# zyang1580/SML

Measured on AMD Instinct MI355X. Metric: SML retrain-period training triples/s (MF + transfer stages), Yelp-shaped synthetic, d=32, higher is better.
Workload: dtype f32; 1 GPU; yelp_period: users=60000 items=123000 interactions/period=75000 neg=999 d=32 multi_num=10 MF_batch=1024 TR_batch=256 val_eval=True (the reference's 40 validation evaluations per period: 31 computed on the GPU, 9 memoised because the tables did not change in between -- identical numbers); MF stage: the transfer net runs once per DISTINCT row of a batch (the reference gathers one row per occurrence:; parallelism=single GPU

## Files before the change

sml_amd/csrc/transfer_fwd_body.inc:

```
    constexpr int R = SML_TM * MT;
    constexpr int K1 = SML_C2 * D;
    constexpr int HL = SML_HID / NS / HSEQ;
    constexpr int S1 = K1 + 4;
    constexpr int S2 = HL + 4;
    constexpr int KS1 = K1 / 16;
    constexpr int EPT = R * D / 512;
    constexpr int JT = D / 16;
    constexpr int CT = HL / 16 / 8;
    constexpr int KL = HL / 16;
    constexpr int KSPL = (D == 32) ? 8 : (D == 64 ? 4 : 2);
    constexpr int JSPL = 8 / KSPL;
    constexpr int JTW = JT / JSPL;
    constexpr int KPW = KL / KSPL;
    static_assert(CT >= 1 && KPW >= 1 && MT * NS <= 4 && (R * D) % 512 == 0, "tiling");
    constexpr int REG0 = cmax(R * S1, KSPL * R * (D + 1));
    __shared__ __attribute__((aligned(16))) float smem[REG0 + cmax(R * S2, R * (D + 1) + R) + 104];
    __shared__ SmlSched swin[SML_SW];
    __shared__ SmlReplayEnt rtab[MT == 1 ? SML_RP_N : 1];
    float* A1s = smem;
    float* a2s = smem + REG0;
    float* cws = smem + REG0 + cmax(R * S2, R * (D + 1) + R);
    float* xts = a2s;
    float* nrm = a2s + R * (D + 1);
    float* part = smem;

    const int tid = threadIdx.x, lane = tid & 63, wv = tid >> 6, l15 = lane & 15, g4 = lane >> 4;
    TL_BEGIN(NS == 4 ? 1 : 4); TL_PREV();
    constexpr int WT_LOCAL = (NS == 4) ? SML_WT_FWD : SML_WT_FWD_LOCAL;
    int tile, h;
    if constexpr (NS == 4) {
        const int x = (int)blockIdx.x % 8;
        h = x / 2; tile = 2 * ((int)blockIdx.x / 8) + (x % 2);
        if (tile >= a.tiles_total) return;
// ... 2 lines not shown
    const SmlSeg sg = sidx ? a.seg[1] : a.seg[0];
    const int row0 = (tile - (sidx ? a.tiles0 : 0)) * R;
    const float* __restrict__ theta = sg.theta;
    float cw_reg = 0.0f;
    constexpr bool CONVSTEP = (NS == 4 && MT == 1 && HSEQ == 1);
    const bool cstep = CONVSTEP && a.cs_in != nullptr;
    constexpr int CRG = 21, CC4 = SML_CG / 4;
    f32x4 cg_acc = {0.f, 0.f, 0.f, 0.f}, cgx[4];
    float cs_p = 0.f, cs_m = 0.f, cs_v = 0.f;
    const int cs_k = tid;
    const int cs_off = cs_k < 30 ? cs_k : cs_k < 40 ? cs_k + 2 : cs_k < 90 ? cs_k + 4 : cs_k + 6;
    const int cg_lo = sidx ? a.cg_split : 0, cg_hi = sidx ? a.cg_total : a.cg_split;
    int cg_t = 0;
    const bool cg_mine = CONVSTEP && cstep && a.cg_part != nullptr && tid < CRG * CC4;
    if (!cstep) { if (tid < 104) cw_reg = theta[tid]; }
    const bool lazy = sg.last_tab != nullptr;
    if (lazy) sched_window_load(swin, a.sched, a.cur_step - 1, tid);
    const bool closed = MT == 1 && lazy && a.sched_len > 0;
    if constexpr (MT == 1) { if (closed) replay_table_build(rtab, a.sched, a.sched_len, a.cur_step - 1, tid); }
    const bool saver = (h == 0);

    constexpr bool PRE = (CT == 1) && (KS1 / 2 <= 5) && HSEQ == 1;
    constexpr int PF2 = KPW < 4 ? KPW : 4;
    const f32x4* __restrict__ img1 = reinterpret_cast<const f32x4*>(sg.pk + sml_pk_p1(D));
    const f32x4* __restrict__ img2 = reinterpret_cast<const f32x4*>(sg.pk + sml_pk_p2(D));
    const int tile0 = h * (HL / 16) + wv * CT;
    const int kq = wv % KSPL, jq = wv / KSPL;
    auto t1 = [tile0](int) { return tile0; };
    auto k1 = [](int t) { return t * (KS1 / 2); };
    auto t2 = [jq](int t) { return jq * JTW + t; };
    auto nokofs = [](int) { return 0; };
// ... 27 lines not shown
        if (dense) {
            const int live = (int)sg.hdr[tile - (sidx ? a.tiles0 : 0)].nrows;
#pragma unroll
            for (int q = 0; q < EPT; ++q) {
                const int r = (q * 512 + tid) / D;
                const uint32_t trow = sg.drec[row0 + r].row;
                ok[q] = r < live;
                idx[q] = ok[q] ? (int64_t)trow : 0;
            }
            if (live == 0) return;
        } else {
#pragma unroll
            for (int q = 0; q < EPT; ++q) {
                const int row = row0 + (q * 512 + tid) / D;
                ok[q] = row < sg.n_rows;
                idx[q] = ok[q] ? seg_row_index(sg, row) : 0;
            }
        }
        if constexpr (CONVSTEP) {
            if (cstep) {
                if (tid < 95) {
                    const float* st_ = a.cs_in + (int64_t)sidx * 3 * SML_CG;
                    cs_p = st_[cs_k]; cs_m = st_[SML_CG + cs_k]; cs_v = st_[2 * SML_CG + cs_k];
                }
                if (cg_mine) {
                    const int rg = tid / CC4, c4 = tid % CC4;
                    cg_t = rg + (cg_lo > rg ? ((cg_lo - rg + CRG - 1) / CRG) * CRG : 0);
#pragma unroll
                    for (int u = 0; u < 4; ++u) {
                        const int t = cg_t + u * CRG;
                        cgx[u] = *reinterpret_cast<const f32x4*>(a.cg_part + (int64_t)(t < cg_hi ? t : cg_lo) * SML_CG + c4 * 4);
                    }
                }
                __builtin_amdgcn_sched_barrier(0);
            }
        }
#pragma unroll
        for (int q = 0; q < EPT; ++q) {
            const int w = (q * 512 + tid) % D;
            xt[q] = sg.xt_tab[idx[q] * D + w];
            xh[q] = sg.xh_tab[idx[q] * D + w];
        }
        float m[EPT], v[EPT];
        int from[EPT];
        if (lazy) {
#pragma unroll
            for (int q = 0; q < EPT; ++q) {
                const int w = (q * 512 + tid) % D;
                m[q] = sg.m_tab[idx[q] * D + w];
                v[q] = sg.v_tab[idx[q] * D + w];
                from[q] = sg.last_tab[idx[q]];
            }
        }
        if constexpr (PREW) {
            ring_preload<CT, 5>(ringw1, img1, KS1, 0, lane, tw, nokofs);
            ring_preload<JTW, PF2>(ringw2, img2, 32, h * KL + kq * KPW, lane, t2, nokofs);
        }
        if constexpr (CONVSTEP) {
            if (cstep) {
                __builtin_amdgcn_sched_barrier(0);
                float* P = smem;
                if (tid < CRG * CC4) {
                    const int rg = tid / CC4, c4 = tid % CC4;
                    if (cg_mine) {
#pragma unroll
                        for (int u = 0; u < 4; ++u) if (cg_t + u * CRG < cg_hi) cg_acc += cgx[u];
                        for (int t0 = cg_t + 4 * CRG; t0 < cg_hi; t0 += 4 * CRG) {
                            f32x4 x[4];
#pragma unroll
                            for (int u = 0; u < 4; ++u) {
                                const int t = t0 + u * CRG;
                                x[u] = *reinterpret_cast<const f32x4*>(a.cg_part + (int64_t)(t < cg_hi ? t : cg_lo) * SML_CG + c4 * 4);
                            }
#pragma unroll
                            for (int u = 0; u < 4; ++u) if (t0 + u * CRG < cg_hi) cg_acc += x[u];
                        }
                    }
                    *reinterpret_cast<f32x4*>(P + rg * SML_CG + c4 * 4) = cg_acc;
                }
                asm volatile("s_waitcnt lgkmcnt(0)\n\ts_barrier" ::: "memory");
                if (tid < 95) {
// ... 187 lines not shown
```

sml_amd/csrc/transfer_net.hip:

```cpp
#include <cstdlib>
#include "sml_dev.h"
#include "sml_kernels.h"

#ifdef SML_TIMELINE
__device__ long long* g_timeline = nullptr;
#ifndef SML_TL_SECOND
#define SML_TL_SECOND (gridDim.x - 1)
#endif
#define TL_BEGIN(KID) long long* tl_rec = nullptr; const int tl_all = 70000 + (KID) * 1024; { if (g_timeline && threadIdx.x == 0) g_timeline[tl_all + 512 + blockIdx.x] = wall_clock64(); } { long long* tl = g_timeline; if (tl && threadIdx.x == 0 && (blockIdx.x == 0 || blockIdx.x == SML_TL_SECOND)) { \
    const unsigned long long slot = atomicAdd(reinterpret_cast<unsigned long long*>(tl), 1ull); tl_rec = tl + 16 + slot * 16; tl_rec[0] = (KID) * 2 + (blockIdx.x != 0); tl_rec[1] = wall_clock64(); for (int q = 2; q < 16; ++q) tl_rec[q] = 0; } }
#define TL(i) do { if (tl_rec) tl_rec[(i)] = wall_clock64(); } while (0)
#define TL_DONE() do { long long* tl = g_timeline; if (tl && threadIdx.x == 0) { const long long now_ = wall_clock64(); \
    atomicMax(reinterpret_cast<unsigned long long*>(tl + 2), (unsigned long long)now_); tl[tl_all + blockIdx.x] = now_; } } while (0)
#define TL_PREV() do { if (tl_rec) tl_rec[8] = (long long)__hip_atomic_load(reinterpret_cast<unsigned long long*>(g_timeline + 2), __ATOMIC_RELAXED, __HIP_MEMORY_SCOPE_AGENT); } while (0)
#else
#define TL_BEGIN(KID) const int tl_all = 0; (void)tl_all; long long* const tl_rec = nullptr; (void)tl_rec
#define TL(i) do { } while (0)
#define TL_DONE() do { } while (0)
#define TL_PREV() do { } while (0)
#endif
#ifndef SML_WT_FWD
#define SML_WT_FWD 2
#endif
#ifndef SML_WT_BWD
// ... 34 lines not shown
    }
#pragma unroll
    for (int q = 0; q < SML_C2; ++q) {
        float s = cw[SML_OFF_C2B + q];
#pragma unroll
        for (int c = 0; c < SML_C1; ++c) s += cw[SML_OFF_C2W + q * SML_C1 + c] * o.h1[c];
        o.h2p[q] = s;
    }
}

__device__ __forceinline__ int64_t seg_row_index(const SmlSeg& s, int r) {
    if (s.tri == nullptr) return r;
    if (!s.is_item) return s.tri[(int64_t)r * 3];
    return r < s.B ? s.tri[(int64_t)r * 3 + 1] : s.tri[(int64_t)(r - s.B) * 3 + 2];
}

template <int NT, int PFD, typename TileOf, typename KOfs>
__device__ __forceinline__ void ring_preload(f32x4 (&ring)[PFD][NT], const f32x4* __restrict__ bimg, int ksteps_total, int ks0,
                                             int lane, TileOf tile_of, KOfs kofs) {
#pragma unroll
    for (int i = 0; i < PFD; ++i)
#pragma unroll
        for (int t = 0; t < NT; ++t) ring[i][t] = bimg[(tile_of(t) * ksteps_total + ks0 + kofs(t) + i) * 64 + lane];
    __builtin_amdgcn_sched_barrier(0x86);
}

template <int MT, int NT, int NK, int PFD, bool SPLITK, typename TileOf, typename KOfs>
__device__ __forceinline__ void mma16_ring(f32x4 (&acc)[MT][NT], f32x4 (&ring)[PFD][NT], const float* arow, int a_mt,
                                           const f32x4* __restrict__ bimg, int ksteps_total, int ks0, int lane,
                                           TileOf tile_of, KOfs kofs) {
// ... 67 lines not shown
constexpr int cmax(int a, int b) { return a > b ? a : b; }

#define SML_FWD_HOT_PARAMS const float* __restrict__ p_pk, const float* __restrict__ p_theta, const int64_t* __restrict__ p_tri,             \
                           const float* __restrict__ p_cs_in, const float* __restrict__ p_cg_part, int p_B, int p_n0, int p_tiles, int p_cg
#define SML_FWD_HOT_PATCH(a, D)                                                                                                               \
    (a).tiles0 = p_tiles & 0x7fffffff; (a).tiles_total = (p_tiles & 0x7fffffff) + (p_tiles < 0 ? (2 * p_B + SML_TM - 1) / SML_TM : 0);       \
    (a).cs_in = p_cs_in; (a).cg_part = p_cg_part; (a).cg_split = p_cg & 0x7fff; (a).cg_total = (p_cg >> 15) & 0xffff;                         \
    (a).seg[0].pk = p_pk; (a).seg[1].pk = p_pk + sml_pk_size(D); (a).seg[0].theta = p_theta; (a).seg[1].theta = p_theta + sml_net_size(D); \
    (a).seg[0].tri = p_tri; (a).seg[1].tri = p_tri; (a).seg[0].B = p_B; (a).seg[1].B = p_B; (a).seg[0].n_rows = p_n0;                        \
    (a).seg[1].n_rows = p_n0 == p_B ? 2 * p_B : ((2 * p_B + SML_TM - 1) / SML_TM) * SML_TM;                                                   \
    (a).seg[0].is_item = 0; (a).seg[1].is_item = 1
template <int D, int MT, int NS, int HSEQ = 1>
__global__ __launch_bounds__(512) __attribute__((amdgpu_waves_per_eu(HSEQ > 1 ? 4 : 2, HSEQ > 1 ? 4 : 2))) void k_transfer_fwd(SML_FWD_HOT_PARAMS, SmlFwdArgs a_in) {
    SmlFwdArgs a = a_in;
    SML_FWD_HOT_PATCH(a, D);
#include "transfer_fwd_body.inc"
}
template <int D>
__global__ __launch_bounds__(512) __attribute__((amdgpu_waves_per_eu(4, 4))) void k_side_transfer_fwd(SmlFwdArgs a) {
    constexpr int MT = 2, NS = 1, HSEQ = 2;
#include "transfer_fwd_body.inc"
}

typedef __bf16 bf16x8 __attribute__((ext_vector_type(8)));
__device__ __forceinline__ f32x4 mfma_bf(const uint4& a, const uint4& b, f32x4 c) {
    return __builtin_amdgcn_mfma_f32_16x16x32_bf16(__builtin_bit_cast(bf16x8, a), __builtin_bit_cast(bf16x8, b), c, 0, 0, 0);
}
__device__ __forceinline__ uint32_t bf16_rne(float x) {
    uint32_t u = __float_as_uint(x);
    u += 0x7fffu + ((u >> 16) & 1u);
    return u >> 16;
}
__device__ __forceinline__ void split3(float x, unsigned short& h, unsigned short& m, unsigned short& l) {
    const uint32_t a = bf16_rne(x);
    const float r1 = x - __uint_as_float(a << 16);
// ... 213 lines not shown
    __shared__ __attribute__((aligned(16))) unsigned short A2b[3][R][S2B];
    __shared__ float cws[104];
    __shared__ SmlSched swin[SML_SW];
    __shared__ SmlReplayEnt rtab[SML_RP_N];
    float* part = reinterpret_cast<float*>(&A2b[0][0][0]);
    static_assert(sizeof(A2b) >= 8 * R * (D + 1) * sizeof(float), "part fits");
    const int tid = threadIdx.x, lane = tid & 63, wv = tid >> 6, l15 = lane & 15, g4 = lane >> 4;
    const int tile = (int)blockIdx.x;
    const int sidx = tile >= a.tiles0;
    const SmlSeg sg = sidx ? a.seg[1] : a.seg[0];
    const int tl = tile - (sidx ? a.tiles0 : 0);
    const int row0 = tl * R;
    const float* __restrict__ theta = sg.theta;
    const unsigned short* __restrict__ p1x = pkx + (int64_t)sidx * sml_bx3_size(D) + sml_bx3_p1(D);
    const unsigned short* __restrict__ p2x = pkx + (int64_t)sidx * sml_bx3_size(D) + sml_bx3_p2(D);
    if (tid < 104) cws[tid] = theta[tid];
    const bool lazy = sg.last_tab != nullptr;
    if (lazy) sched_window_load(swin, a.sched, a.cur_step - 1, tid);
    const int r = tid / D, w = tid % D;
    bool ok; int64_t idx;
    if (sg.drec != nullptr) {
        const int live = (int)sg.hdr[tl].nrows;
        const uint32_t trow = sg.drec[row0 + r].row;
        ok = r < live; idx = ok ? (int64_t)trow : 0;
        if (live == 0) return;
    } else {
        ok = row0 + r < sg.n_rows;
        idx = ok ? seg_row_index(sg, row0 + r) : 0;
    }
    float xt = sg.xt_tab[idx * D + w], xh = sg.xh_tab[idx * D + w];
    float m = 0.0f, v = 0.0f; int from = -1;
    if (lazy) { m = sg.m_tab[idx * D + w]; v = sg.v_tab[idx * D + w]; from = sg.last_tab[idx]; }
    const bool closed = lazy && a.sched_len > 0;
    if (closed) replay_table_build(rtab, a.sched, a.sched_len, a.cur_step - 1, tid);
    uint4 bw[2][CT][3];
    auto load_b1 = [&](int ks, uint4 (&dst)[CT][3]) {
#pragma unroll
        for (int t = 0; t < CT; ++t)
#pragma unroll
            for (int p = 0; p < 3; ++p)
                dst[t][p] = *reinterpret_cast<const uint4*>(p1x + ((((int64_t)(wv * CT + t) * KS1 + ks) * 3 + p) * 64 + lane) * 8);
    };
    load_b1(0, bw[0]);
    float bias1[CT];
#pragma unroll
    for (int t = 0; t < CT; ++t) bias1[t] = theta[sml_off_f1b(D) + (wv * CT + t) * 16 + l15];
    const float bias2 = theta[sml_off_f2b(D) + w];
    __builtin_amdgcn_sched_barrier(0);
    if (!ok) { xt = 1.0f; xh = 0.0f; }
    float nr2 = xt * xt;
#pragma unroll
    for (int off = D / 2; off >= 1; off >>= 1) nr2 += __shfl_xor(nr2, off, 64);
    __syncthreads();
    if (lazy) {
        if (ok) adam_replay_t(xh, m, v, from, a.cur_step - 1, a.sched, swin, a.cur_step - 1, closed ? rtab : nullptr);
        if (sg.mrep != nullptr) {
            sg.mrep[(int64_t)(row0 + r) * D + w] = ok ? m : 0.0f;
            sg.vrep[(int64_t)(row0 + r) * D + w] = ok ? v : 0.0f;
        }
    }
    {
        const float xc = a.k2 ? 0.0f : (xt * xh) / sqrtf(nr2);
        Pro p;
        conv_prologue(cws, xt, xh, xc, p);
#pragma unroll
        for (int c = 0; c < SML_C2; ++c) {
            unsigned short h, mm, l;
// ... 210 lines not shown
    __shared__ __attribute__((aligned(16))) float Cs[DENSEOK ? SML_TILE_ENT * D : 4];
    __shared__ uint32_t rlen[16], rstart[17];
    __shared__ float Ps[DENSEOK ? 512 : 4];
    float* dZs = smem;
    float* dOs = smem + R * S2;
    float* part = smem;
    float* cws = smem + SZ;

    const int tid = threadIdx.x, lane = tid & 63, wv = tid >> 6, l15 = lane & 15, g4 = lane >> 4;
    TL_BEGIN(5); TL_PREV();
    const int sidx = (int)blockIdx.x >= p_tiles0;
    const SmlBwdSeg& sg = a.seg[sidx];
    const float* __restrict__ sg_theta = p_theta + (sidx ? sml_net_size(D) : 0);
    const int row0 = ((int)blockIdx.x - (sidx ? p_tiles0 : 0)) * R;
    if (p_world > 0 && (int)blockIdx.x >= p_tiles_live) { peer_signal(a.push); return; }
    if (tid < 104) cws[tid] = sg_theta[tid];
#ifndef SML_PREB
#define SML_PREB 0
#endif
    constexpr bool PREB = (SML_PREB != 0) && (MT == 1) && (D <= 32);
    const f32x4* __restrict__ p2b = reinterpret_cast<const f32x4*>(sg.pk + sml_pk_p2b(D));
    const f32x4* __restrict__ p1b = reinterpret_cast<const f32x4*>(sg.pk + sml_pk_p1b(D));
    auto tileA2 = [wv](int t) { return wv * 4 + t; };
    auto tileA1 = [wv](int t) { return (wv / KSPL) * 5 + t; };
    auto nokofs = [](int) { return 0; };
    f32x4 ringb2[PREB ? KSD : 1][4], ringb1[PREB ? 4 : 1][5];
    float zpre[PREB ? MT : 1][4][4];
    auto preload_operands = [&]() {
        if constexpr (PREB) {
            ring_preload<4, KSD>(ringb2, p2b, KSD, 0, lane, tileA2, nokofs);
            ring_preload<5, 4>(ringb1, p1b, 32, (wv % KSPL) * KPER, lane, tileA1, nokofs);
// ... 219 lines not shown
    }
    constexpr bool PRELOAD = (EPT == 1);
    float x0p = 0.f, x1p = 0.f, x2p = 0.f;
    if (PRELOAD) {
        const float* x = sg.xin + (int64_t)(row0 + tid / D) * 3 * D;
        x0p = x[tid % D]; x1p = x[D + tid % D]; x2p = x[2 * D + tid % D];
    }
    constexpr bool FUSABLE = D <= 64;
    const bool fused = FUSABLE && a.fu.slot_info != nullptr;
    FusedPre fpre;
    fpre.info = SML_SLOT_ONCE; fpre.trow = 0; fpre.m = fpre.v = 0.0f; fpre.r0 = make_uint4(0u, 0u, 0u, 0u); fpre.r1 = fpre.r0;
    if constexpr (FUSABLE && PRELOAD) {
        if (fused) fused_prefetch<D>(a, sidx, row0 + tid / D, tid % D, row0 + tid / D < sg.n_rows, fpre);
        if (dense) dense_prefetch<D>(a, sidx, row0 + tid / D, tid % D, tid / D < live, fpre);
    }
    __syncthreads();
    TL(2);
    {
        f32x4 acc[MT][4];
        zero_acc(acc);
        float z[MT][4][4];
#pragma unroll
        for (int t = 0; t < 4; ++t)
#pragma unroll
            for (int mt = 0; mt < MT; ++mt)
#pragma unroll
                for (int q = 0; q < 4; ++q)
                    z[mt][t][q] = PREB ? zpre[mt][t][q] : sg.z1[(int64_t)(row0 + mt * SML_TM + 4 * g4 + q) * SML_HID + (wv * 4 + t) * 16 + l15];
        if constexpr (PREB) mma16_ring<MT, 4, KSD, KSD, false>(acc, ringb2, dOs + l15 * SD + 4 * g4, SML_TM * SD, p2b, KSD, 0, lane, tileA2, nokofs);
        else mma16_rows<MT, 4, KSD, KSD>(acc, dOs + l15 * SD + 4 * g4, SML_TM * SD, p2b, KSD, 0, lane, tileA2);
// ... 346 lines not shown
        if (lane == 0) lred[wv] = v;
    }
    __syncthreads();
    if (tid == 0) {
        float sacc = 0.0f;
#pragma unroll
        for (int w8 = 0; w8 < 8; ++w8) sacc += lred[w8];
        a.loss_part[blockIdx.x] = sacc;
        TL(7);
    }
    TL_DONE();
}

template <int D>
__global__ __launch_bounds__(512) void k_tr_bwd_head(const float* __restrict__ p_out_all, const float* __restrict__ p_z1, const float* __restrict__ p_pk,
                                                     long long p_out_pstride, int p_B, int p_ioff, int p_tiles0, int p_tiles_total, int p_out_np, SmlBwdArgs a) {
    constexpr int R = SML_TM;
    constexpr int HS = 4;
    constexpr int SD = D + 4;
    constexpr int KSD = D / 16;
    constexpr int EPT = R * D / 512;
    static_assert(SML_HID / 16 / HS == 8, "one dA2 column tile per wave");
    __shared__ __attribute__((aligned(16))) float smem[cmax(R * SD, 3 * R * (D + 1))];
    __shared__ float cf[4][SML_TM];
    __shared__ float lred[8];
    float* dOs = smem;
    float* O3 = smem;
    const int tid = threadIdx.x, lane = tid & 63, wv = tid >> 6, l15 = lane & 15, g4 = lane >> 4;
    TL_BEGIN(2); TL_PREV();
    const int x8 = (int)blockIdx.x % 8;
    const int hs = x8 / 2, tile = 2 * ((int)blockIdx.x / 8) + (x8 % 2);
    if (tile >= p_tiles_total) return;
    const int sidx = tile >= p_tiles0;
    const SmlBwdSeg sg = sidx ? a.seg[1] : a.seg[0];
    const int row0 = (tile - (sidx ? p_tiles0 : 0)) * R;
    const int n_rows = sidx ? 2 * p_B : p_B;
    const float* __restrict__ z1_seg = p_z1 + (sidx ? (int64_t)p_ioff * SML_HID : 0);
    const f32x4* __restrict__ p2b = reinterpret_cast<const f32x4*>(p_pk + (sidx ? sml_pk_size(D) : 0) + sml_pk_p2b(D));
    const int ct = hs * 8 + wv;
    float vu[EPT][SML_FWD_NS], vi[EPT][SML_FWD_NS], vn[EPT][SML_FWD_NS];
#pragma unroll
    for (int q = 0; q < EPT; ++q) {
        const int e = q * 512 + tid, r = e / D, w = e % D;
        const int row = row0 + r;
        const bool inr = row < n_rows;
        const int t = !inr ? 0 : ((sidx && row >= p_B) ? row - p_B : row);
        const float* pu = p_out_all + (int64_t)t * D + w;
        const float* pi = p_out_all + (int64_t)(p_ioff + t) * D + w;
        const float* pn = p_out_all + (int64_t)(p_ioff + p_B + t) * D + w;
#pragma unroll
        for (int p = 0; p < SML_FWD_NS; ++p) {
            const int64_t po = (int64_t)min(p, p_out_np - 1) * p_out_pstride;
            vu[q][p] = pu[po]; vi[q][p] = pi[po]; vn[q][p] = pn[po];
        }
    }
    float z[4];
#pragma unroll
    for (int q = 0; q < 4; ++q) z[q] = z1_seg[(int64_t)(row0 + 4 * g4 + q) * SML_HID + ct * 16 + l15];
    f32x4 ring[KSD];
#pragma unroll
    for (int ks = 0; ks < KSD; ++ks) ring[ks] = p2b[(ct * KSD + ks) * 64 + lane];
    float ou[EPT], oi[EPT], on[EPT];
#pragma unroll
    for (int q = 0; q < EPT; ++q) {
        const int e = q * 512 + tid, r = e / D, w = e % D;
        const float inr = (row0 + r < n_rows) ? 1.0f : 0.0f;
        ou[q] = oi[q] = on[q] = 0.0f;
#pragma unroll
        for (int p = 0; p < SML_FWD_NS; ++p) {
            const float live = p < p_out_np ? inr : 0.0f;
            ou[q] += live * vu[q][p]; oi[q] += live * vi[q][p]; on[q] += live * vn[q][p];
        }
        if constexpr (D > 64) {
            O3[(0 * R + r) * (D + 1) + w] = ou[q];
            O3[(1 * R + r) * (D + 1) + w] = oi[q];
            O3[(2 * R + r) * (D + 1) + w] = on[q];
// ... 27 lines not shown
#pragma unroll
        for (int q = 0; q < EPT; ++q) {
            const int e = q * 512 + tid, r = e / D, w = e % D;
            const int row = row0 + r;
            float sp = ou[q] * oi[q], sn = ou[q] * on[q], uu = ou[q] * ou[q];
#pragma unroll
            for (int off = D / 2; off >= 1; off >>= 1) {
                sp += __shfl_xor(sp, off, 64); sn += __shfl_xor(sn, off, 64); uu += __shfl_xor(uu, off, 64);
            }
            float lt, d0, d1, inv_nu, cc;
            coeffs(sp, sn, uu, lt, d0, d1, inv_nu, cc);
            d0 *= a.scale; d1 *= a.scale;
            if (!sidx && hs == 0 && w == 0 && row < n_rows) lsum += lt * a.scale;
            const float g = dout_of(row, d0, d1, inv_nu, cc, ou[q], oi[q], on[q]);
            dOs[r * SD + w] = g;
            if (hs == 0) st_out<SML_WT_BWD>(&sg.dout[(int64_t)row * D + w], g);
        }
    } else {
        __syncthreads();
        if (tid < R) {
            float sp = 0.f, sn = 0.f, uu = 0.f;
#pragma unroll 8
            for (int w = 0; w < D; ++w) {
                const float u = O3[(0 * R + tid) * (D + 1) + w];
                sp += u * O3[(1 * R + tid) * (D + 1) + w];
                sn += u * O3[(2 * R + tid) * (D + 1) + w];
                uu += u * u;
            }
            float lt, d0, d1, inv_nu, cc;
            coeffs(sp, sn, uu, lt, d0, d1, inv_nu, cc);
            cf[0][tid] = d0 * a.scale; cf[1][tid] = d1 * a.scale; cf[2][tid] = inv_nu; cf[3][tid] = cc;
            if (!sidx && hs == 0 && row0 + tid < n_rows) lsum = lt * a.scale;
        }
        __syncthreads();
#pragma unroll
        for (int q = 0; q < EPT; ++q) {
            const int e = q * 512 + tid, r = e / D, w = e % D;
            const int row = row0 + r;
            const float g = dout_of(row, cf[0][r], cf[1][r], cf[2][r], cf[3][r], ou[q], oi[q], on[q]);
            dOs[r * SD + w] = g;
            if (hs == 0) st_out<SML_WT_BWD>(&sg.dout[(int64_t)row * D + w], g);
        }
    }
    __syncthreads();
    TL(2);
    {
        f32x4 acc = {0.f, 0.f, 0.f, 0.f};
#pragma unroll
        for (int ks = 0; ks < KSD; ++ks) {
            const f32x4 av = *reinterpret_cast<const f32x4*>(dOs + l15 * SD + 4 * g4 + ks * 16);
#pragma unroll
            for (int e = 0; e < 4; ++e) acc = mfma16(av[e], ring[ks][e], acc);
        }
        const int n = ct * 16 + l15;
#pragma unroll
        for (int q = 0; q < 4; ++q)
            st_out<SML_WT_BWD>(&sg.dz1[(int64_t)(row0 + 4 * g4 + q) * SML_HID + n], acc[q] * sml_gelu_grad(z[q]));
    }
    TL(3);
    {
        float v = lsum;
#pragma unroll
        for (int off = 32; off >= 1; off >>= 1) v += __shfl_xor(v, off, 64);
        if (lane == 0) lred[wv] = v;
    }
    __syncthreads();
    if (tid == 0) {
        float sacc = 0.0f;
#pragma unroll
        for (int w8 = 0; w8 < 8; ++w8) sacc += lred[w8];
        a.loss_part[tile * HS + hs] = sacc;
        TL(7);
    }
    TL_DONE();
}

template <int D>
__device__ __forceinline__ void pack_store(float* __restrict__ pk, int off, float p) {
    constexpr int K1 = SML_C2 * D;
    if (off >= SML_OFF_F1W && off < sml_off_f1b(D)) {
        const int n = (off - SML_OFF_F1W) / K1, k = (off - SML_OFF_F1W) % K1;
        pk[sml_pk_p1(D) + pk_pos(K1 / 16, n, k)] = p;
        pk[sml_pk_p1b(D) + pk_pos(SML_HID / 16, k, n)] = p;
    } else if (off >= sml_off_f2w(D) && off < sml_off_f2b(D)) {
        const int j = (off - sml_off_f2w(D)) / SML_HID, n = (off - sml_off_f2w(D)) % SML_HID;
        pk[sml_pk_p2(D) + pk_pos(SML_HID / 16, j, n)] = p;
        pk[sml_pk_p2b(D) + pk_pos(D / 16, n, j)] = p;
    }
}

#define SML_WG_TILE_SMEM (8 * 32 * 33 + 8 * 32 + 32 * 33)
template <int D>
__device__ __forceinline__ void wgrad_tile(const SmlWgArgs& a, const SmlWgSeg& sg, int xcd, int kk, float* smem_wg, long long* tl_rec) {
    constexpr int K1 = SML_C2 * D;
    constexpr int KT = K1 / 32;
    constexpr int JT = D / 32;
    constexpr int T1 = 16 * KT, T2 = JT * 16, TN = T1 + T2;
    constexpr int NS = sml_net_size(D);
    float* part = smem_wg;
    float* csum = smem_wg + 8 * 32 * 33;
    float* wt = csum + 8 * 32;
    const int tid = threadIdx.x, lane = tid & 63, wv = tid >> 6, l31 = lane & 31, hi = lane >> 5;
    const bool fuse = a.theta != nullptr;
    SmlSched sc; sc.step_size = a.step_size; sc.bc2_sqrt = a.bc2_sqrt;
    static_assert(TN % 8 == 0 && T2 == 16 * JT, "tile map");
    constexpr int PER = 2 * (KT + JT);
    const int net = 1 - kk / PER, rr = kk % PER;
    const bool is_w1 = rr < 2 * KT;
    int ti, tj;
    if (is_w1) { ti = 2 * xcd + rr / KT; tj = rr % KT; } else { tj = 2 * xcd + (rr - 2 * KT) / JT; ti = (rr - 2 * KT) % JT; }
    const float* __restrict__ Asrc = is_w1 ? sg.dz1 : sg.dout;
    const int lda = is_w1 ? SML_HID : D;
    const float* __restrict__ Bsrc = is_w1 ? sg.a1 : sg.a2;
    const int ldb = is_w1 ? K1 : SML_HID;
    const bool gelu_b = !is_w1 && a.gelu_b != 0;
    int woff[2];
    float wp[2] = {0.f, 0.f}, wm[2] = {0.f, 0.f}, wvv[2] = {0.f, 0.f};
#pragma unroll
    for (int q = 0; q < 2; ++q) {
        const int e = q * 512 + tid, i = e >> 5, j = e & 31;
        woff[q] = is_w1 ? SML_OFF_F1W + (ti * 32 + i) * K1 + tj * 32 + j
                        : sml_off_f2w(D) + (ti * 32 + i) * SML_HID + tj * 32 + j;
    }
    const bool has_bias = (tj == 0 && tid < 32);
    const int boff = is_w1 ? sml_off_f1b(D) + ti * 32 + tid : sml_off_f2b(D) + ti * 32 + tid;
    float bp = 0.f, bm = 0.f, bv2 = 0.f;
    f32x16 acc;
#pragma unroll
    for (int q = 0; q < 16; ++q) acc[q] = 0.0f;
    float colsum = 0.0f;
// ... 106 lines not shown
template <int D>
__global__ __launch_bounds__(512) __attribute__((amdgpu_waves_per_eu(4, 4))) void k_tr_wgrad2(const float* __restrict__ p_dz1, const float* __restrict__ p_a1,
        const float* __restrict__ p_dout, const float* __restrict__ p_a2, const float* __restrict__ p_pk_net, const float* __restrict__ p_xin, int p_B, int p_n_tail,
        SmlWgArgs a) {
    SmlWgSeg seg0 = a.seg[0], seg1 = a.seg[1];
    {
        const int64_t slot1 = (int64_t)SML_R * ((p_B + SML_R - 1) / SML_R);
        seg0.dz1 = p_dz1; seg1.dz1 = p_dz1 + slot1 * SML_HID;
        seg0.a1 = p_a1; seg1.a1 = p_a1 + slot1 * SML_C2 * D;
        seg0.dout = p_dout; seg1.dout = p_dout + slot1 * D;
        seg0.a2 = p_a2; seg1.a2 = p_a2 + slot1 * SML_HID;
        seg0.pk_net = p_pk_net; seg1.pk_net = p_pk_net + sml_pk_size(D);
        seg0.xin = p_xin; seg1.xin = p_xin + slot1 * 3 * D;
        seg0.n_rows = p_B; seg1.n_rows = 2 * p_B;
    }
    const int h_n_tail = p_n_tail, h_tiles0 = (p_B + SML_TM - 1) / SML_TM, h_tiles_total = h_tiles0 + (2 * p_B + SML_TM - 1) / SML_TM;
    constexpr int R = SML_TM;
    constexpr int CS = D / 16;
    constexpr int S2 = SML_HID + 4;
    constexpr int PSTR = SML_C2 * 16 + 1;
    constexpr int CGS = 20;
    constexpr int SZ0 = cmax(cmax(R * S2, 8 * R * PSTR), 2 * 256 * CGS);
    constexpr int TAIL_SMEM = SZ0 + 104 + 8 * 256;
    constexpr int NS = sml_net_size(D);
    __shared__ __attribute__((aligned(16))) float smem[cmax(TAIL_SMEM, SML_WG_TILE_SMEM)];
    __shared__ int s_last;
    TL_BEGIN(3); TL_PREV();
    const int tid = threadIdx.x, lane = tid & 63, wv = tid >> 6, l15 = lane & 15, g4 = lane >> 4;
    if ((int)blockIdx.x >= h_n_tail) {
        const int vb = (int)blockIdx.x - h_n_tail;
        const SmlWgSeg sgt = ((vb / 8) / (2 * (SML_C2 * D / 32 + D / 32))) ? SmlWgSeg(seg0) : SmlWgSeg(seg1);
        float* const smem_tile = smem + (vb * 3 - vb - vb - vb);
        wgrad_tile<D>(a, sgt, (int)blockIdx.x % 8, vb / 8, smem_tile, tl_rec);
        TL_DONE();
        return;
    }
    float* part = smem;
    float* cgA = smem;
    float* cgB = smem + 256 * CGS;
    float* cws = smem + SZ0;
    float* red = smem + SZ0 + 104;
    const int tb = (int)blockIdx.x;
    const int tile = tb / CS, cs = tb % CS;
    const bool live = tile < h_tiles_total;
    if (live) {
        const int sidx = tile >= h_tiles0;
        const SmlWgSeg sg = sidx ? seg1 : seg0;
        const int row0 = (tile - (sidx ? h_tiles0 : 0)) * R;
// ... 278 lines not shown
        else k_side_transfer_fwd<64><<<dim3(tiles_total), dim3(512), 0, st>>>(a);
        return hipGetLastError();
    }
    const SmlSeg& s0 = a.seg[0]; const SmlSeg& s1 = a.seg[1];
    const bool two = tiles_total > a.tiles0 && s1.n_rows > 0;
    const int tt = a.tiles_total > a.tiles0 ? a.tiles_total : a.tiles0;
    const int n1 = s0.n_rows == s0.B ? 2 * s0.B : ((2 * s0.B + SML_TM - 1) / SML_TM) * SML_TM;
    if ((s0.tri != nullptr && s0.is_item != 0) || a.cg_split < 0 || a.cg_split > 0x7fff || a.cg_total < 0 || a.cg_total > 0xffff ||
        a.tiles0 < 0 || (tt != a.tiles0 && tt != a.tiles0 + (2 * s0.B + SML_TM - 1) / SML_TM) ||
        (two && (s1.pk != s0.pk + sml_pk_size(d) || s1.theta != s0.theta + sml_net_size(d) || s1.tri != s0.tri || s1.B != s0.B || s1.n_rows != n1 ||
                 (s1.tri != nullptr && s1.is_item != 1))))
        return hipErrorInvalidValue;
#define SML_FWD_HOT_ARGS s0.pk, s0.theta, s0.tri, a.cs_in, a.cg_part, s0.B, s0.n_rows, (int)((unsigned)a.tiles0 | (tt != a.tiles0 ? 0x80000000u : 0u)), \
                         (a.cg_split | (a.cg_total << 15)), a
    if (mt == 1 && ns == 1) { SML_DISPATCH_D(d, k_transfer_fwd<DD, 1, 1><<<dim3(tiles_total), dim3(512), 0, st>>>(SML_FWD_HOT_ARGS)); }
    else if (mt == 1 && ns == 4) { SML_DISPATCH_D(d, k_transfer_fwd<DD, 1, 4><<<dim3(((tiles_total + 1) / 2) * 8), dim3(512), 0, st>>>(SML_FWD_HOT_ARGS)); }
    else if (mt == 1 && ns == 2) { SML_DISPATCH_D(d, k_transfer_fwd<DD, 1, 2><<<dim3(tiles_total * 2), dim3(512), 0, st>>>(SML_FWD_HOT_ARGS)); }
    else if (mt == 2 && ns == 1) {
        if (d == 32) k_transfer_fwd<32, 2, 1, 2><<<dim3(tiles_total), dim3(512), 0, st>>>(SML_FWD_HOT_ARGS);
        else if (d == 64) k_transfer_fwd<64, 2, 1, 2><<<dim3(tiles_total), dim3(512), 0, st>>>(SML_FWD_HOT_ARGS);
        else if (d == 128) k_transfer_fwd<128, 2, 1><<<dim3(tiles_total), dim3(512), 0, st>>>(SML_FWD_HOT_ARGS);
        else return hipErrorInvalidValue;
    }
    else return hipErrorInvalidValue;
#undef SML_FWD_HOT_ARGS
    return hipGetLastError();
}
hipError_t sml_launch_bwd(int d, int split, const SmlBwdArgs& a, int tiles_total, hipStream_t st) {
    if (tiles_total <= 0) return hipSuccess;
    if (split) {
// ... 1 lines not shown
        if (d == 32) k_transfer_bwd<32, true><<<dim3(grid), dim3(512), 0, st>>>(a);
        else if (d == 64) k_transfer_bwd<64, false><<<dim3(grid), dim3(512), 0, st>>>(a);
        else if (d == 128) k_transfer_bwd<128, false><<<dim3(grid), dim3(512), 0, st>>>(a);
        else return hipErrorInvalidValue;
    } else {
        if (a.seg[1].theta != a.seg[0].theta + sml_net_size(d)) return hipErrorInvalidValue;
        SML_DISPATCH_D(d, k_transfer_bwd_full<DD, 1><<<dim3(tiles_total), dim3(512), 0, st>>>(a.dn.hdr, a.dn.ent, a.seg[0].theta, a.out_all, a.tiles0, a.push.world,
                                                                                                a.tiles_live, a.B, a));
    }
    return hipGetLastError();
}
hipError_t sml_launch_tr_bwd_head(int d, const SmlBwdArgs& a, int tiles_total, hipStream_t st) {
    if (tiles_total <= 0) return hipSuccess;
    const SmlBwdSeg& s0 = a.seg[0]; const SmlBwdSeg& s1 = a.seg[1];
    if (s1.z1 != s0.z1 + (int64_t)a.ioff * SML_HID || s1.pk != s0.pk + sml_pk_size(d) || s0.n_rows != a.B || s1.n_rows != 2 * a.B ||
        s0.is_item != 0 || s1.is_item != 1)
        return hipErrorInvalidValue;
    SML_DISPATCH_D(d, k_tr_bwd_head<DD><<<dim3(((tiles_total + 1) / 2) * 8), dim3(512), 0, st>>>(a.out_all, a.seg[0].z1, a.seg[0].pk, (long long)a.out_pstride,
                                                                                                   a.B, a.ioff, a.tiles0, a.tiles_total, a.out_np, a));
    return hipGetLastError();
}
int sml_wgrad_tiles(int d) { return 2 * (16 * (SML_C2 * d / 32) + (d / 32) * 16); }
hipError_t sml_launch_tr_wgrad2(int d, const SmlWgArgs& a, hipStream_t st) {
    const int tiles = sml_wgrad_tiles(d);
    const SmlWgSeg& s0 = a.seg[0]; const SmlWgSeg& s1 = a.seg[1];
    const int B = s0.n_rows;
    const int64_t slot1 = (int64_t)SML_R * ((B + SML_R - 1) / SML_R);
    if (s1.n_rows != 2 * B || s1.dz1 != s0.dz1 + slot1 * SML_HID || s1.a1 != s0.a1 + slot1 * SML_C2 * d || s1.dout != s0.dout + slot1 * d ||
        s1.a2 != s0.a2 + slot1 * SML_HID || s1.pk_net != s0.pk_net + sml_pk_size(d) || s1.xin != s0.xin + slot1 * 3 * d ||
        a.tiles0 != (B + SML_TM - 1) / SML_TM || a.tiles_total != a.tiles0 + (2 * B + SML_TM - 1) / SML_TM)
        return hipErrorInvalidValue;
    SML_DISPATCH_D(d, k_tr_wgrad2<DD><<<dim3(a.n_tail + tiles), dim3(512), 0, st>>>(s0.dz1, s0.a1, s0.dout, s0.a2, s0.pk_net, s0.xin, B, a.n_tail, a));
    return hipGetLastError();
}
hipError_t sml_launch_theta_adam(int d, const SmlThetaAdamArgs& a, hipStream_t st) {
    const int n = 2 * sml_net_size(d) / 4;
    if (a.peer.world > 0) { SML_DISPATCH_D(d, k_theta_adam<DD, true><<<dim3((n + 255) / 256), dim3(256), 0, st>>>(a)); }
    else { SML_DISPATCH_D(d, k_theta_adam<DD, false><<<dim3((n + 255) / 256), dim3(256), 0, st>>>(a)); }
    return hipGetLastError();
}
__global__ __launch_bounds__(256) void k_conv_state_init(const float* __restrict__ theta, const float* __restrict__ m, const float* __restrict__ v,
                                                         int net_size, float* __restrict__ cs) {
    const int net = threadIdx.x >> 7, k = threadIdx.x & 127;
    if (k >= 95) return;
    const int off = k < 30 ? k : k < 40 ? k + 2 : k < 90 ? k + 4 : k + 6;
    const long long i = (long long)net * net_size + off;
    float* o = cs + net * 3 * SML_CG;
// ... 48 lines not shown
```

Before: 15.98 million triples/s.

## Add non-lazy transfer forward kernel and hoist scalar arg loads earlier

Adds a k_tr_fwd specialization used when neither segment has lazy Adam tables. It drops the replay table and schedule window, issues row-index and conv-state/cg-part loads unconditionally with dummy addresses so they are in flight early, and picks the result afterwards. It also packs kind, scale and gelu_b into scalar kernel parameters, and moves theta and schedule loads into registers so the shared-memory stores sit just before the barrier. The aim is to cut load latency and kernel-argument memory reads, at the cost of more code paths and some wasted speculative loads.

```diff
diff --git a/sml_amd/csrc/transfer_fwd_body.inc b/sml_amd/csrc/transfer_fwd_body.inc
--- a/sml_amd/csrc/transfer_fwd_body.inc
+++ b/sml_amd/csrc/transfer_fwd_body.inc
@@ -16,7 +16,7 @@
     constexpr int REG0 = cmax(R * S1, KSPL * R * (D + 1));
     __shared__ __attribute__((aligned(16))) float smem[REG0 + cmax(R * S2, R * (D + 1) + R) + 104];
     __shared__ SmlSched swin[SML_SW];
-    __shared__ SmlReplayEnt rtab[MT == 1 ? SML_RP_N : 1];
+    __shared__ SmlReplayEnt rtab[(MT == 1 && !NOLAZY) ? SML_RP_N : 1];
     float* A1s = smem;
     float* a2s = smem + REG0;
     float* cws = smem + REG0 + cmax(R * S2, R * (D + 1) + R);
@@ -49,7 +49,7 @@
     int cg_t = 0;
     const bool cg_mine = CONVSTEP && cstep && a.cg_part != nullptr && tid < CRG * CC4;
     if (!cstep) { if (tid < 104) cw_reg = theta[tid]; }
-    const bool lazy = sg.last_tab != nullptr;
+    const bool lazy = !NOLAZY && sg.last_tab != nullptr;
     if (lazy) sched_window_load(swin, a.sched, a.cur_step - 1, tid);
     const bool closed = MT == 1 && lazy && a.sched_len > 0;
     if constexpr (MT == 1) { if (closed) replay_table_build(rtab, a.sched, a.sched_len, a.cur_step - 1, tid); }
@@ -107,26 +107,32 @@
             for (int q = 0; q < EPT; ++q) {
                 const int row = row0 + (q * 512 + tid) / D;
                 ok[q] = row < sg.n_rows;
-                idx[q] = ok[q] ? seg_row_index(sg, row) : 0;
+                if constexpr (NOLAZY) idx[q] = seg_row_index_load(sg, ok[q] ? row : 0, reinterpret_cast<const int64_t*>(img1));
+                else idx[q] = ok[q] ? seg_row_index(sg, row) : 0;
             }
         }
         if constexpr (CONVSTEP) {
-            if (cstep) {
-                if (tid < 95) {
-                    const float* st_ = a.cs_in + (int64_t)sidx * 3 * SML_CG;
-                    cs_p = st_[cs_k]; cs_m = st_[SML_CG + cs_k]; cs_v = st_[2 * SML_CG + cs_k];
-                }
-                if (cg_mine) {
-                    const int rg = tid / CC4, c4 = tid % CC4;
-                    cg_t = rg + (cg_lo > rg ? ((cg_lo - rg + CRG - 1) / CRG) * CRG : 0);
-#pragma unroll
-                    for (int u = 0; u < 4; ++u) {
-                        const int t = cg_t + u * CRG;
-                        cgx[u] = *reinterpret_cast<const f32x4*>(a.cg_part + (int64_t)(t < cg_hi ? t : cg_lo) * SML_CG + c4 * 4);
-                    }
+            {
+                const bool cg_on = cstep && a.cg_part != nullptr && cg_hi > cg_lo;
+                const float* nowhere = reinterpret_cast<const float*>(img1);
+                const float* st_ = cstep ? a.cs_in + (int64_t)sidx * 3 * SML_CG : nowhere;
+                const int ck = min(cs_k, 94);
+                cs_p = st_[ck]; cs_m = st_[SML_CG + ck]; cs_v = st_[2 * SML_CG + ck];
+                const int rg = min(tid / CC4, CRG - 1), c4 = tid % CC4;
+                cg_t = rg + (cg_lo > rg ? ((cg_lo - rg + CRG - 1) / CRG) * CRG : 0);
+                const float* cgp = cg_on ? a.cg_part : nowhere;
+                const int hi_c = cg_on ? cg_hi : 0, lo_c = cg_on ? cg_lo : 0;
+#pragma unroll
+                for (int u = 0; u < 4; ++u) {
+                    const int t = cg_t + u * CRG;
+                    cgx[u] = *reinterpret_cast<const f32x4*>(cgp + (int64_t)(t < hi_c ? t : lo_c) * SML_CG + c4 * 4);
                 }
                 __builtin_amdgcn_sched_barrier(0);
             }
+        }
+        if constexpr (NOLAZY) {
+#pragma unroll
+            for (int q = 0; q < EPT; ++q) idx[q] = seg_row_index_pick(sg, ok[q] ? row0 + (q * 512 + tid) / D : 0, idx[q]);
         }
 #pragma unroll
         for (int q = 0; q < EPT; ++q) {
@@ -150,14 +156,15 @@
             ring_preload<JTW, PF2>(ringw2, img2, 32, h * KL + kq * KPW, lane, t2, nokofs);
         }
         if constexpr (CONVSTEP) {
+            __builtin_amdgcn_sched_barrier(0);
+#pragma unroll
+            for (int u = 0; u < 4; ++u) cg_acc = (cg_mine && cg_t + u * CRG < cg_hi) ? cg_acc + cgx[u] : cg_acc;
+            asm volatile("" : "+v"(cg_acc));
             if (cstep) {
-                __builtin_amdgcn_sched_barrier(0);
                 float* P = smem;
                 if (tid < CRG * CC4) {
                     const int rg = tid / CC4, c4 = tid % CC4;
                     if (cg_mine) {
-#pragma unroll
-                        for (int u = 0; u < 4; ++u) if (cg_t + u * CRG < cg_hi) cg_acc += cgx[u];
                         for (int t0 = cg_t + 4 * CRG; t0 < cg_hi; t0 += 4 * CRG) {
                             f32x4 x[4];
 #pragma unroll
diff --git a/sml_amd/csrc/transfer_net.hip b/sml_amd/csrc/transfer_net.hip
--- a/sml_amd/csrc/transfer_net.hip
+++ b/sml_amd/csrc/transfer_net.hip
@@ -72,6 +72,12 @@
     if (!s.is_item) return s.tri[(int64_t)r * 3];
     return r < s.B ? s.tri[(int64_t)r * 3 + 1] : s.tri[(int64_t)(r - s.B) * 3 + 2];
 }
+__device__ __forceinline__ int64_t seg_row_index_load(const SmlSeg& s, int r, const int64_t* somewhere) {
+    const bool id = s.tri == nullptr;
+    const int64_t o = !s.is_item ? (int64_t)r * 3 : (r < s.B ? (int64_t)r * 3 + 1 : (int64_t)(r - s.B) * 3 + 2);
+    return (id ? somewhere : s.tri)[id ? 0 : o];
+}
+__device__ __forceinline__ int64_t seg_row_index_pick(const SmlSeg& s, int r, int64_t loaded) { return s.tri == nullptr ? (int64_t)r : loaded; }
 
 template <int NT, int PFD, typename TileOf, typename KOfs>
 __device__ __forceinline__ void ring_preload(f32x4 (&ring)[PFD][NT], const f32x4* __restrict__ bimg, int ksteps_total, int ks0,
@@ -169,11 +175,21 @@
 __global__ __launch_bounds__(512) __attribute__((amdgpu_waves_per_eu(HSEQ > 1 ? 4 : 2, HSEQ > 1 ? 4 : 2))) void k_transfer_fwd(SML_FWD_HOT_PARAMS, SmlFwdArgs a_in) {
     SmlFwdArgs a = a_in;
     SML_FWD_HOT_PATCH(a, D);
+    constexpr bool NOLAZY = false;
+#include "transfer_fwd_body.inc"
+}
+template <int D>
+__global__ __launch_bounds__(512) __attribute__((amdgpu_waves_per_eu(2, 2))) void k_tr_fwd(SML_FWD_HOT_PARAMS, SmlFwdArgs a_in) {
+    SmlFwdArgs a = a_in;
+    SML_FWD_HOT_PATCH(a, D);
+    constexpr int MT = 1, NS = 4, HSEQ = 1;
+    constexpr bool NOLAZY = true;
 #include "transfer_fwd_body.inc"
 }
 template <int D>
 __global__ __launch_bounds__(512) __attribute__((amdgpu_waves_per_eu(4, 4))) void k_side_transfer_fwd(SmlFwdArgs a) {
     constexpr int MT = 2, NS = 1, HSEQ = 2;
+    constexpr bool NOLAZY = false;
 #include "transfer_fwd_body.inc"
 }
 
@@ -417,14 +433,17 @@
     const float* __restrict__ theta = sg.theta;
     const unsigned short* __restrict__ p1x = pkx + (int64_t)sidx * sml_bx3_size(D) + sml_bx3_p1(D);
     const unsigned short* __restrict__ p2x = pkx + (int64_t)sidx * sml_bx3_size(D) + sml_bx3_p2(D);
-    if (tid < 104) cws[tid] = theta[tid];
+    const float cw_reg = theta[tid < 104 ? tid : 103];
     const bool lazy = sg.last_tab != nullptr;
-    if (lazy) sched_window_load(swin, a.sched, a.cur_step - 1, tid);
+    const int sw_k = a.cur_step - SML_SW + (tid < SML_SW ? tid : SML_SW - 1);
+    SmlSched sw_reg; sw_reg.step_size = 0.0f; sw_reg.bc2_sqrt = 0.0f;
     const int r = tid / D, w = tid % D;
     bool ok; int64_t idx;
-    if (sg.drec != nullptr) {
-        const int live = (int)sg.hdr[tl].nrows;
-        const uint32_t trow = sg.drec[row0 + r].row;
+    const bool dn = sg.drec != nullptr;
+    int live = 0; uint32_t trow = 0;
+    if (dn) { live = (int)sg.hdr[tl].nrows; trow = sg.drec[row0 + r].row; }
+    if (lazy) sw_reg = a.sched[sw_k >= 0 ? sw_k : 0];
+    if (dn) {
         ok = r < live; idx = ok ? (int64_t)trow : 0;
         if (live == 0) return;
     } else {
@@ -454,6 +473,8 @@
     float nr2 = xt * xt;
 #pragma unroll
     for (int off = D / 2; off >= 1; off >>= 1) nr2 += __shfl_xor(nr2, off, 64);
+    if (tid < 104) cws[tid] = cw_reg;
+    if (lazy && tid < SML_SW && sw_k >= 0) swin[tid] = sw_reg;
     __syncthreads();
     if (lazy) {
         if (ok) adam_replay_t(xh, m, v, from, a.cur_step - 1, a.sched, swin, a.cur_step - 1, closed ? rtab : nullptr);
@@ -694,7 +715,7 @@
     const float* __restrict__ sg_theta = p_theta + (sidx ? sml_net_size(D) : 0);
     const int row0 = ((int)blockIdx.x - (sidx ? p_tiles0 : 0)) * R;
     if (p_world > 0 && (int)blockIdx.x >= p_tiles_live) { peer_signal(a.push); return; }
-    if (tid < 104) cws[tid] = sg_theta[tid];
+    const float cw_reg = sg_theta[tid < 104 ? tid : 103];
 #ifndef SML_PREB
 #define SML_PREB 0
 #endif
@@ -944,6 +965,7 @@
         if (fused) fused_prefetch<D>(a, sidx, row0 + tid / D, tid % D, row0 + tid / D < sg.n_rows, fpre);
         if (dense) dense_prefetch<D>(a, sidx, row0 + tid / D, tid % D, tid / D < live, fpre);
     }
+    if (tid < 104) cws[tid] = cw_reg;
     __syncthreads();
     TL(2);
     {
@@ -1320,7 +1342,11 @@
 
 template <int D>
 __global__ __launch_bounds__(512) void k_tr_bwd_head(const float* __restrict__ p_out_all, const float* __restrict__ p_z1, const float* __restrict__ p_pk,
-                                                     long long p_out_pstride, int p_B, int p_ioff, int p_tiles0, int p_tiles_total, int p_out_np, SmlBwdArgs a) {
+                                                     long long p_out_pstride, int p_B, int p_ioff, int p_tiles0, int p_tiles_total, int p_np_kind, float p_scale,
+                                                     SmlBwdArgs a_in) {
+    SmlBwdArgs a = a_in;
+    a.kind = p_np_kind >> 8; a.scale = p_scale;
+    const int p_out_np = p_np_kind & 0xff;
     constexpr int R = SML_TM;
     constexpr int HS = 4;
     constexpr int SD = D + 4;
@@ -1338,7 +1364,6 @@
     const int hs = x8 / 2, tile = 2 * ((int)blockIdx.x / 8) + (x8 % 2);
     if (tile >= p_tiles_total) return;
     const int sidx = tile >= p_tiles0;
-    const SmlBwdSeg sg = sidx ? a.seg[1] : a.seg[0];
     const int row0 = (tile - (sidx ? p_tiles0 : 0)) * R;
     const int n_rows = sidx ? 2 * p_B : p_B;
     const float* __restrict__ z1_seg = p_z1 + (sidx ? (int64_t)p_ioff * SML_HID : 0);
@@ -1366,6 +1391,9 @@
     f32x4 ring[KSD];
 #pragma unroll
     for (int ks = 0; ks < KSD; ++ks) ring[ks] = p2b[(ct * KSD + ks) * 64 + lane];
+    float* const dout_p = sidx ? a.seg[1].dout : a.seg[0].dout;
+    float* const dz1_p = sidx ? a.seg[1].dz1 : a.seg[0].dz1;
+    float* const loss_p = a.loss_part;
     float ou[EPT], oi[EPT], on[EPT];
 #pragma unroll
     for (int q = 0; q < EPT; ++q) {
@@ -1423,7 +1451,7 @@
             if (!sidx && hs == 0 && w == 0 && row < n_rows) lsum += lt * a.scale;
             const float g = dout_of(row, d0, d1, inv_nu, cc, ou[q], oi[q], on[q]);
             dOs[r * SD + w] = g;
-            if (hs == 0) st_out<SML_WT_BWD>(&sg.dout[(int64_t)row * D + w], g);
+            if (hs == 0) st_out<SML_WT_BWD>(&dout_p[(int64_t)row * D + w], g);
         }
     } else {
         __syncthreads();
@@ -1448,7 +1476,7 @@
             const int row = row0 + r;
             const float g = dout_of(row, cf[0][r], cf[1][r], cf[2][r], cf[3][r], ou[q], oi[q], on[q]);
             dOs[r * SD + w] = g;
-            if (hs == 0) st_out<SML_WT_BWD>(&sg.dout[(int64_t)row * D + w], g);
+            if (hs == 0) st_out<SML_WT_BWD>(&dout_p[(int64_t)row * D + w], g);
         }
     }
     __syncthreads();
@@ -1464,7 +1492,7 @@
         const int n = ct * 16 + l15;
 #pragma unroll
         for (int q = 0; q < 4; ++q)
-            st_out<SML_WT_BWD>(&sg.dz1[(int64_t)(row0 + 4 * g4 + q) * SML_HID + n], acc[q] * sml_gelu_grad(z[q]));
+            st_out<SML_WT_BWD>(&dz1_p[(int64_t)(row0 + 4 * g4 + q) * SML_HID + n], acc[q] * sml_gelu_grad(z[q]));
     }
     TL(3);
     {
@@ -1478,7 +1506,7 @@
         float sacc = 0.0f;
 #pragma unroll
         for (int w8 = 0; w8 < 8; ++w8) sacc += lred[w8];
-        a.loss_part[tile * HS + hs] = sacc;
+        loss_p[tile * HS + hs] = sacc;
         TL(7);
     }
     TL_DONE();
@@ -1500,7 +1528,7 @@
 
 #define SML_WG_TILE_SMEM (8 * 32 * 33 + 8 * 32 + 32 * 33)
 template <int D>
-__device__ __forceinline__ void wgrad_tile(const SmlWgArgs& a, const SmlWgSeg& sg, int xcd, int kk, float* smem_wg, long long* tl_rec) {
+__device__ __forceinline__ void wgrad_tile(const SmlWgArgs& a, const SmlWgSeg& sg, bool a_gelu_b, int xcd, int kk, float* smem_wg, long long* tl_rec) {
     constexpr int K1 = SML_C2 * D;
     constexpr int KT = K1 / 32;
     constexpr int JT = D / 32;
@@ -1522,7 +1550,7 @@
     const int lda = is_w1 ? SML_HID : D;
     const float* __restrict__ Bsrc = is_w1 ? sg.a1 : sg.a2;
     const int ldb = is_w1 ? K1 : SML_HID;
-    const bool gelu_b = !is_w1 && a.gelu_b != 0;
+    const bool gelu_b = !is_w1 && a_gelu_b;
     int woff[2];
     float wp[2] = {0.f, 0.f}, wm[2] = {0.f, 0.f}, wvv[2] = {0.f, 0.f};
 #pragma unroll
@@ -1659,7 +1687,7 @@
         seg0.xin = p_xin; seg1.xin = p_xin + slot1 * 3 * D;
         seg0.n_rows = p_B; seg1.n_rows = 2 * p_B;
     }
-    const int h_n_tail = p_n_tail, h_tiles0 = (p_B + SML_TM - 1) / SML_TM, h_tiles_total = h_tiles0 + (2 * p_B + SML_TM - 1) / SML_TM;
+    const int h_n_tail = p_n_tail & 0x3fffffff, h_tiles0 = (p_B + SML_TM - 1) / SML_TM, h_tiles_total = h_tiles0 + (2 * p_B + SML_TM - 1) / SML_TM;
     constexpr int R = SML_TM;
     constexpr int CS = D / 16;
     constexpr int S2 = SML_HID + 4;
@@ -1676,7 +1704,7 @@
         const int vb = (int)blockIdx.x - h_n_tail;
         const SmlWgSeg sgt = ((vb / 8) / (2 * (SML_C2 * D / 32 + D / 32))) ? SmlWgSeg(seg0) : SmlWgSeg(seg1);
         float* const smem_tile = smem + (vb * 3 - vb - vb - vb);
-        wgrad_tile<D>(a, sgt, (int)blockIdx.x % 8, vb / 8, smem_tile, tl_rec);
+        wgrad_tile<D>(a, sgt, (p_n_tail & 0x40000000) != 0, (int)blockIdx.x % 8, vb / 8, smem_tile, tl_rec);
         TL_DONE();
         return;
     }
@@ -1985,6 +2013,9 @@
 #define SML_FWD_HOT_ARGS s0.pk, s0.theta, s0.tri, a.cs_in, a.cg_part, s0.B, s0.n_rows, (int)((unsigned)a.tiles0 | (tt != a.tiles0 ? 0x80000000u : 0u)), \
                          (a.cg_split | (a.cg_total << 15)), a
     if (mt == 1 && ns == 1) { SML_DISPATCH_D(d, k_transfer_fwd<DD, 1, 1><<<dim3(tiles_total), dim3(512), 0, st>>>(SML_FWD_HOT_ARGS)); }
+    else if (mt == 1 && ns == 4 && s0.last_tab == nullptr && s1.last_tab == nullptr) {
+        SML_DISPATCH_D(d, k_tr_fwd<DD><<<dim3(((tiles_total + 1) / 2) * 8), dim3(512), 0, st>>>(SML_FWD_HOT_ARGS));
+    }
     else if (mt == 1 && ns == 4) { SML_DISPATCH_D(d, k_transfer_fwd<DD, 1, 4><<<dim3(((tiles_total + 1) / 2) * 8), dim3(512), 0, st>>>(SML_FWD_HOT_ARGS)); }
     else if (mt == 1 && ns == 2) { SML_DISPATCH_D(d, k_transfer_fwd<DD, 1, 2><<<dim3(tiles_total * 2), dim3(512), 0, st>>>(SML_FWD_HOT_ARGS)); }
     else if (mt == 2 && ns == 1) {
@@ -2016,10 +2047,11 @@
     if (tiles_total <= 0) return hipSuccess;
     const SmlBwdSeg& s0 = a.seg[0]; const SmlBwdSeg& s1 = a.seg[1];
     if (s1.z1 != s0.z1 + (int64_t)a.ioff * SML_HID || s1.pk != s0.pk + sml_pk_size(d) || s0.n_rows != a.B || s1.n_rows != 2 * a.B ||
-        s0.is_item != 0 || s1.is_item != 1)
+        s0.is_item != 0 || s1.is_item != 1 || a.out_np < 0 || a.out_np > 0xff || a.kind < 0 || a.kind > 0xffff)
         return hipErrorInvalidValue;
     SML_DISPATCH_D(d, k_tr_bwd_head<DD><<<dim3(((tiles_total + 1) / 2) * 8), dim3(512), 0, st>>>(a.out_all, a.seg[0].z1, a.seg[0].pk, (long long)a.out_pstride,
-                                                                                                   a.B, a.ioff, a.tiles0, a.tiles_total, a.out_np, a));
+                                                                                                   a.B, a.ioff, a.tiles0, a.tiles_total, a.out_np | (a.kind << 8),
+                                                                                                   a.scale, a));
     return hipGetLastError();
 }
 int sml_wgrad_tiles(int d) { return 2 * (16 * (SML_C2 * d / 32) + (d / 32) * 16); }
@@ -2030,9 +2062,10 @@
     const int64_t slot1 = (int64_t)SML_R * ((B + SML_R - 1) / SML_R);
     if (s1.n_rows != 2 * B || s1.dz1 != s0.dz1 + slot1 * SML_HID || s1.a1 != s0.a1 + slot1 * SML_C2 * d || s1.dout != s0.dout + slot1 * d ||
         s1.a2 != s0.a2 + slot1 * SML_HID || s1.pk_net != s0.pk_net + sml_pk_size(d) || s1.xin != s0.xin + slot1 * 3 * d ||
-        a.tiles0 != (B + SML_TM - 1) / SML_TM || a.tiles_total != a.tiles0 + (2 * B + SML_TM - 1) / SML_TM)
+        a.tiles0 != (B + SML_TM - 1) / SML_TM || a.tiles_total != a.tiles0 + (2 * B + SML_TM - 1) / SML_TM || a.n_tail < 0 || a.n_tail >= 0x40000000)
         return hipErrorInvalidValue;
-    SML_DISPATCH_D(d, k_tr_wgrad2<DD><<<dim3(a.n_tail + tiles), dim3(512), 0, st>>>(s0.dz1, s0.a1, s0.dout, s0.a2, s0.pk_net, s0.xin, B, a.n_tail, a));
+    SML_DISPATCH_D(d, k_tr_wgrad2<DD><<<dim3(a.n_tail + tiles), dim3(512), 0, st>>>(s0.dz1, s0.a1, s0.dout, s0.a2, s0.pk_net, s0.xin, B,
+                                                                                     a.n_tail | (a.gelu_b ? 0x40000000 : 0), a));
     return hipGetLastError();
 }
 hipError_t sml_launch_theta_adam(int d, const SmlThetaAdamArgs& a, hipStream_t st) {
```

Result: no change. 16.13 million triples/s (median of 6 runs) (+0.9%).
